# g-benton/Volt

Hardware: AMD Instinct MI355X
Metric: mll_grad_steps_per_s (higher is better)
Workload: dtype f32; 1 GPU; MLL+grad step, N=4096, batch=64 series per GPU, Volatility kernel + EWMA(k=25) mean; series_total=64, parallelism=series-sharded x1, collective=none

## Files before the change

### volt_amd/csrc/tiles.h

```cpp
#pragma once
#include "common.h"
#include "host.h"

namespace volt {


__device__ __forceinline__ float input_elem(const KSource& src, const float* Kb, float add, const float* Ab, int Np,
                                            bool usek, int gi, int gj) {
    if (usek) {
        float v = (gi < src.N && gj < src.N) ? Kb[(int64_t)gi * src.ldk + gj] : 0.f;
        if (gi == gj) v = (gi < src.N) ? v + add : 1.f;
        return v;
    }
    return Ab[(int64_t)gi * Np + gj];
}

template <bool FROMK, int ABL = 0, bool CHASE = false, bool LOCALP = false>
__device__ __forceinline__ void update_body(float* __restrict__ A, int Np, int rowblk, int colblk, int kb0, int kb1,
                                            bool fromk, int b, const KSource& src, float* smem,
                                            bool to_image = false, const Chase* ch = nullptr, bool* ch_ok = nullptr) {
    float* Ab = A + (int64_t)b * Np * Np;
    const float* Arows = Ab + (int64_t)rowblk * TS * Np + (int64_t)kb0 * TS;
    const float* Brows = Ab + (int64_t)colblk * TS * Np + (int64_t)kb0 * TS;
    const int lane = threadIdx.x & 63, wave = threadIdx.x >> 6;
    const int wr = wave >> 1, wc = wave & 1;
    float* C = Ab + (int64_t)rowblk * TS * Np + (int64_t)colblk * TS;
    f32x16 acc[4];
    const bool usek = FROMK && fromk;
    const float add = usek ? ((src.sigma2 ? src.sigma2[b] : 0.f) + src.jitter) : 0.f;
    const float* Kb = usek ? src.K + (int64_t)b * src.bsk : nullptr;
#pragma unroll
    for (int tm = 0; tm < 2; ++tm)
#pragma unroll
        for (int tn = 0; tn < 2; ++tn)
#pragma unroll
            for (int q = 0; q < 16; ++q) {
                const int r = wr * 64 + tm * 32 + accrow(q, lane);
                const int c = wc * 64 + tn * 32 + (lane & 31);
                if (ABL & 1) acc[tm * 2 + tn][q] = 0.f;
                else acc[tm * 2 + tn][q] = -input_elem(src, Kb, add, Ab, Np, usek, rowblk * TS + r, colblk * TS + c);
            }
    gemm_nt_128<0, CHASE, LOCALP>(Arows, Np, Brows, Np, (kb1 - kb0) * (TS / BK), acc, smem, ch, ch_ok);
    if (ABL & 2) {
        float sum = 0.f;
#pragma unroll
        for (int t4 = 0; t4 < 4; ++t4)
#pragma unroll
            for (int q = 0; q < 16; ++q) sum += acc[t4][q];
        C[(int64_t)(threadIdx.x >> 1) * Np + (threadIdx.x & 1)] = sum;
        return;
    }
    if (to_image) {
        __syncthreads();
#pragma unroll
        for (int tm = 0; tm < 2; ++tm)
#pragma unroll
            for (int tn = 0; tn < 2; ++tn)
#pragma unroll
                for (int q = 0; q < 16; ++q) {
                    const int r = wr * 64 + tm * 32 + accrow(q, lane);
                    const int c = wc * 64 + tn * 32 + (lane & 31);
                    smem[r * (TS + 1) + c] = (c <= r) ? -acc[tm * 2 + tn][q] : 0.f;
                }
        return;
    }
#pragma unroll
    for (int tm = 0; tm < 2; ++tm)
#pragma unroll
        for (int tn = 0; tn < 2; ++tn)
#pragma unroll
            for (int q = 0; q < 16; ++q) {
                const int r = wr * 64 + tm * 32 + accrow(q, lane);
                const int c = wc * 64 + tn * 32 + (lane & 31);
                C[(int64_t)r * Np + c] = -acc[tm * 2 + tn][q];
            }
}

constexpr int DT = TS + 1;
constexpr int DIAG_LDS_FLOATS = TS * DT;

__device__ __forceinline__ f32x16 mm32_lds_lds(f32x16 acc, const float* __restrict__ A, const float* __restrict__ B) {
    const int lane = threadIdx.x & 63, l31 = lane & 31, lh = lane >> 5;
    float av[16], bv[16];
#pragma unroll
    for (int s2 = 0; s2 < 16; ++s2) {
        const int kk = 2 * s2 + lh;
        av[s2] = A[l31 * DT + kk];
        bv[s2] = B[kk * DT + l31];
    }
    VOLT_SB();
#pragma unroll
    for (int s2 = 0; s2 < 16; ++s2) acc = __builtin_amdgcn_mfma_f32_32x32x2f32(av[s2], bv[s2], acc, 0, 0, 0);
    return acc;
}
__device__ __forceinline__ f32x16 mm32_lds_reg(f32x16 acc, const float* __restrict__ A, const f32x16& Breg) {
    const int lane = threadIdx.x & 63, l31 = lane & 31, lh = lane >> 5;
    float av[16];
#pragma unroll
    for (int q = 0; q < 16; ++q) av[q] = A[l31 * DT + (q & 3) + 8 * (q >> 2) + 4 * lh];
    VOLT_SB();
#pragma unroll
    for (int q = 0; q < 16; ++q) acc = __builtin_amdgcn_mfma_f32_32x32x2f32(av[q], Breg[q], acc, 0, 0, 0);
    return acc;
}

template <bool NEG>
__device__ __forceinline__ f32x16 mm32_nt(f32x16 acc, const float* __restrict__ A, const float* __restrict__ B) {
    const int lane = threadIdx.x & 63, l31 = lane & 31, lh = lane >> 5;
    float av[16], bv[16];
#pragma unroll
    for (int s2 = 0; s2 < 16; ++s2) {
        const int kk = 2 * s2 + lh;
        av[s2] = A[l31 * DT + kk];
        bv[s2] = B[l31 * DT + kk];
    }
    VOLT_SB();
#pragma unroll
    for (int s2 = 0; s2 < 16; ++s2)
        acc = __builtin_amdgcn_mfma_f32_32x32x2f32(NEG ? -av[s2] : av[s2], bv[s2], acc, 0, 0, 0);
    return acc;
}

__device__ __forceinline__ float lane_bcast(float v, int src) {
    return __int_as_float(__builtin_amdgcn_readlane(__float_as_int(v), src));
}

#define VOLT_RL "v_readlane_b32 "
__device__ __forceinline__ void rl_fma3(float& c0, float& c1, float& c2, float b0, float b1, float b2, float s0,
                                        float s1, float s2, int l0, int l1, int l2) {
    float t0, t1, t2;
    asm volatile(VOLT_RL "%3, %9, %12\n\t" VOLT_RL "%4, %10, %13\n\t" VOLT_RL "%5, %11, %14\n\t"
                 "v_fma_f32 %0, -%6, %3, %0\n\tv_fma_f32 %1, -%7, %4, %1\n\tv_fma_f32 %2, -%8, %5, %2"
                 : "+v"(c0), "+v"(c1), "+v"(c2), "=&s"(t0), "=&s"(t1), "=&s"(t2)
                 : "v"(b0), "v"(b1), "v"(b2), "v"(s0), "v"(s1), "v"(s2), "i"(l0), "i"(l1), "i"(l2));
}
__device__ __forceinline__ void rl_fma2(float& c0, float& c1, float b0, float b1, float s0, float s1, int l0, int l1) {
    float t0, t1;
    asm volatile(VOLT_RL "%2, %6, %8\n\t" VOLT_RL "%3, %7, %9\n\ts_nop 0\n\t"
                 "v_fma_f32 %0, -%4, %2, %0\n\tv_fma_f32 %1, -%5, %3, %1"
                 : "+v"(c0), "+v"(c1), "=&s"(t0), "=&s"(t1)
                 : "v"(b0), "v"(b1), "v"(s0), "v"(s1), "i"(l0), "i"(l1));
}
__device__ __forceinline__ void settle(float& v) { asm volatile("s_nop 0" : "+v"(v)); }

__device__ __forceinline__ void rl_fma1(float& c0, float b0, float s0, int l0) {
    float t0;
    asm volatile(VOLT_RL "%1, %3, %4\n\ts_nop 1\n\tv_fma_f32 %0, -%2, %1, %0"
                 : "+v"(c0), "=&s"(t0)
                 : "v"(b0), "v"(s0), "i"(l0));
}

#define VOLT_STAMP(i)                                                                  \
    do {                                                                               \
        if (STAMP && threadIdx.x == 0) stamps[i] = __builtin_amdgcn_s_memtime();       \
    } while (0)

template <int J0, int J1>
__device__ __forceinline__ void pivots16(float (&a)[32], float (&rv)[32], int& npos) {
    settle(a[J0]);
    float d = lane_bcast(a[J0], J0);
    float rinv = __builtin_amdgcn_rsqf(d);
#pragma unroll
    for (int j = J0; j < J1; ++j) {
        npos += (d > 0.f) ? 1 : 0;
        rv[j] = rinv;
        float l = a[j] * rinv;
        settle(l);
        a[j] = l;
        float rnext = 0.f;
        if (j + 1 < J1) {
            rl_fma1(a[j + 1], l, l, j + 1);
            settle(a[j + 1]);
            d = lane_bcast(a[j + 1], j + 1);
            rnext = __builtin_amdgcn_rsqf(d);
        }
        int c = j + 2;
#pragma unroll
        for (; c + 2 < J1; c += 3) rl_fma3(a[c], a[c + 1], a[c + 2], l, l, l, l, l, l, c, c + 1, c + 2);
        if (c + 1 < J1) rl_fma2(a[c], a[c + 1], l, l, l, l, c, c + 1);
        else if (c < J1) rl_fma1(a[c], l, l, c);
        rinv = rnext;
    }
}
template <int R0, int R1>
__device__ __forceinline__ void invert16(const float (&a)[32], const float (&rv)[32], float (&x)[32], int l31) {
#pragma unroll
    for (int r = R0; r < R1; ++r) x[r] = (r == l31) ? 1.f : 0.f;
#pragma unroll
    for (int m = R0; m < R1; ++m) {
        const float xm = x[m] * rv[m];
        x[m] = xm;
        int r = m + 1;
#pragma unroll
        for (; r + 2 < R1; r += 3) rl_fma3(x[r], x[r + 1], x[r + 2], xm, xm, xm, a[m], a[m], a[m], r, r + 1, r + 2);
        if (r + 1 < R1) rl_fma2(x[r], x[r + 1], xm, xm, a[m], a[m], r, r + 1);
        else if (r < R1) rl_fma1(x[r], xm, a[m], r);
    }
}
__device__ __forceinline__ void wave_lds_fence() {
    __builtin_amdgcn_fence(__ATOMIC_RELEASE, "wavefront");
    __builtin_amdgcn_wave_barrier();
    __builtin_amdgcn_fence(__ATOMIC_ACQUIRE, "wavefront");
}

constexpr int PSC = 17;
constexpr int PIVOT_SCRATCH_FLOATS = 2 * 16 * PSC;
static_assert(DIAG_LDS_FLOATS + 3 * PIVOT_SCRATCH_FLOATS <= 2 * STAGE_FLOATS, "pivot scratch must fit behind the image");

template <bool STAMP = false>
__device__ __forceinline__ void pivot_phase(float* __restrict__ sT, int kb, int prow, float (&a)[32], int& npos,
                                            long long* stamps = nullptr) {
    const int lane = threadIdx.x & 63, wave = threadIdx.x >> 6, l31 = lane & 31, l15 = lane & 15, g = lane >> 4;
    const bool panel = prow >= 0;
    const bool prw = panel && lane >= 32;
    const bool low = !prw && l31 >= 16;
    float* Dk = sT + (32 * kb) * DT + 32 * kb;
    float* Rw = prw ? sT + (32 * prow + l31) * DT + 32 * kb : Dk + l31 * DT;
    float* S21 = sT + DIAG_LDS_FLOATS + wave * PIVOT_SCRATCH_FLOATS;
    float* S22 = S21 + 16 * PSC;
    float rv[32];
#pragma unroll
    for (int c = 0; c < 16; ++c) a[c] = Rw[c];
    if (STAMP && kb == 1) VOLT_STAMP(16);
    pivots16<0, 16>(a, rv, npos);
    if (STAMP && kb == 1) VOLT_STAMP(17);
    {
        float* dst = prw ? Rw : S21 + (l31 & 15) * PSC;
        if (prw || low) {
#pragma unroll
            for (int c = 0; c < 16; ++c) dst[c] = a[c];
        }
    }
    wave_lds_fence();
    float v21[4];
#pragma unroll
    for (int s = 0; s < 4; ++s) v21[s] = S21[l15 * PSC + 4 * s + g];
    {
        f32x4 c22;
#pragma unroll
        for (int q = 0; q < 4; ++q) c22[q] = Dk[(16 + 4 * g + q) * DT + 16 + l15];
#pragma unroll
        for (int s = 0; s < 4; ++s) c22 = __builtin_amdgcn_mfma_f32_16x16x4f32(-v21[s], v21[s], c22, 0, 0, 0);
#pragma unroll
        for (int q = 0; q < 4; ++q) S22[(4 * g + q) * PSC + l15] = c22[q];
    }
    if (panel) {
        float* Pk = sT + (32 * prow) * DT + 32 * kb;
#pragma unroll
        for (int t = 0; t < 2; ++t) {
            f32x4 cp;
#pragma unroll
            for (int q = 0; q < 4; ++q) cp[q] = Pk[(16 * t + 4 * g + q) * DT + 16 + l15];
#pragma unroll
            for (int s = 0; s < 4; ++s)
                cp = __builtin_amdgcn_mfma_f32_16x16x4f32(-Pk[(16 * t + l15) * DT + 4 * s + g], v21[s], cp, 0, 0, 0);
#pragma unroll
            for (int q = 0; q < 4; ++q) Pk[(16 * t + 4 * g + q) * DT + 16 + l15] = cp[q];
        }
    }
    wave_lds_fence();
    if (STAMP && kb == 1) VOLT_STAMP(18);
    {
        const float* src = prw ? Rw + 16 : S22 + (l31 & 15) * PSC;
#pragma unroll
        for (int c = 0; c < 16; ++c) {
            const float t = src[c];
            a[16 + c] = (prw || low) ? t : 0.f;
        }
    }
    if (STAMP && kb == 1) VOLT_STAMP(19);
    pivots16<16, 32>(a, rv, npos);
    if (STAMP && kb == 1) VOLT_STAMP(20);
    if (prw) {
#pragma unroll
        for (int c = 16; c < 32; ++c) Rw[c] = a[c];
    }
}

__device__ __forceinline__ __amdgpu_buffer_rsrc_t w_rsrc(float* W) {
    return __builtin_amdgcn_make_buffer_rsrc((void*)W, 0, TS * TS * 4, 0x00020000);
}
template <int AUX = 0>
__device__ __forceinline__ void w_store(__amdgpu_buffer_rsrc_t rs, int voff, int soff, float v) {
    __builtin_amdgcn_raw_buffer_store_b32(__float_as_uint(v), rs, voff, soff, AUX);
}
template <bool SLABS = false>
__device__ __forceinline__ void x_block(float* __restrict__ sT, int kb, __amdgpu_buffer_rsrc_t rs) {
    constexpr int AUX = SLABS ? AUX_SC1 : 0;
    constexpr bool store00 = SLABS;
    const int lane = threadIdx.x & 63, l15 = lane & 15, g = lane >> 4, h = lane >> 5;
    const bool up = (lane & 16) != 0;
    float* Dk = sT + (32 * kb) * DT + 32 * kb;
    const float* Lh = Dk + (16 * h) * DT + 16 * h;
    float v21[4];
#pragma unroll
    for (int s = 0; s < 4; ++s) v21[s] = Dk[(16 + l15) * DT + 4 * s + g];
    float x[16];
#pragma unroll
    for (int r = 0; r < 16; ++r) {
        float acc = (r == l15) ? 1.f : 0.f;
#pragma unroll
        for (int m = 0; m < r; ++m) acc = __builtin_fmaf(-Lh[r * DT + m], x[m], acc);
        const float d = Lh[r * DT + r];
        const float ri = __builtin_amdgcn_rcpf(d);
        x[r] = acc * __builtin_fmaf(__builtin_fmaf(-d, ri, 1.f), ri, ri);
    }
    wave_lds_fence();
    if (!up) {
#pragma unroll
        for (int r = 0; r < 16; ++r) Dk[(16 * h + r) * DT + 16 * h + l15] = x[r];
    }
    wave_lds_fence();
    f32x4 t21 = {0.f, 0.f, 0.f, 0.f}, r21 = {0.f, 0.f, 0.f, 0.f};
#pragma unroll
    for (int s = 0; s < 4; ++s)
        t21 = __builtin_amdgcn_mfma_f32_16x16x4f32(v21[s], Dk[(4 * s + g) * DT + l15], t21, 0, 0, 0);
#pragma unroll
    for (int q = 0; q < 4; ++q)
        r21 = __builtin_amdgcn_mfma_f32_16x16x4f32(Dk[(16 + l15) * DT + 16 + 4 * g + q], t21[q], r21, 0, 0, 0);
    const int wbase = (32 * kb * TS + 32 * kb) * 4;
#pragma unroll
    for (int q = 0; q < 4; ++q) {
        Dk[(16 + 4 * g + q) * DT + l15] = -r21[q];
        w_store<AUX>(rs, wbase + ((16 + 4 * g) * TS + l15) * 4, q * TS * 4, -r21[q]);
    }
    if (!up || h == 0) {
        const int voff = wbase + (up ? 16 + l15 : (16 * h) * TS + 16 * h + l15) * 4;
        if (kb != 0 || lane != 0 || store00) w_store<AUX>(rs, voff, 0, up ? 0.f : x[0]);
#pragma unroll
        for (int r = 1; r < 16; ++r) w_store<AUX>(rs, voff, r * TS * 4, up ? 0.f : x[r]);
    }
}

__device__ __forceinline__ f32x16 zero16() {
    f32x16 z;
#pragma unroll
    for (int q = 0; q < 16; ++q) z[q] = 0.f;
    return z;
}
__device__ __forceinline__ void w_out(__amdgpu_buffer_rsrc_t rs, int i, int j, float* __restrict__ blk, const f32x16& R) {
    const int lane = threadIdx.x & 63;
    const int voff = ((32 * i + 4 * (lane >> 5)) * TS + 32 * j + (lane & 31)) * 4;
#pragma unroll
    for (int q = 0; q < 16; ++q) {
        w_store(rs, voff, ((q & 3) + 8 * (q >> 2)) * TS * 4, -R[q]);
        if (blk) blk[accrow(q, lane) * DT + (lane & 31)] = -R[q];
    }
}

template <bool STAMP = false, bool SLABS = false, bool LOCALPUB = false>
__device__ __forceinline__ void diag_body(float* __restrict__ A, float* __restrict__ Winv, int* __restrict__ info,
                                          int Np, int k, int b, float* smem, long long* stamps = nullptr,
                                          bool loaded = false, int* ready = nullptr, int ready_val = 0,
                                          int* slab = nullptr, int* pre = nullptr) {
    float* sT = smem;
    VOLT_STAMP(0);
    const int n = Np / TS;
    float* D = A + (int64_t)b * Np * Np + (int64_t)k * TS * Np + (int64_t)k * TS;
    float* W = Winv + ((int64_t)b * n + k) * TS * TS;
    const int tid = threadIdx.x;
    const int lane = tid & 63, wave = tid >> 6, l31 = lane & 31;

    if (!loaded) {
        f32x4 v[TS * TS / 4 / NT];
#pragma unroll
        for (int it = 0; it < TS * TS / 4 / NT; ++it) {
            const int e = tid + it * NT, r = e >> 5, c = (e & 31) * 4;
            v[it] = f32x4{0.f, 0.f, 0.f, 0.f};
            if (c <= r) v[it] = *reinterpret_cast<const f32x4*>(D + (int64_t)r * Np + c);
        }
#pragma unroll
        for (int it = 0; it < TS * TS / 4 / NT; ++it) {
            const int e = tid + it * NT, r = e >> 5, c = (e & 31) * 4;
#pragma unroll
            for (int q = 0; q < 4; ++q) sT[r * DT + c + q] = (c + q <= r) ? v[it][q] : 0.f;
        }
    }
    __syncthreads();
    VOLT_STAMP(1);

    auto blk = [&](int i, int j) { return sT + (32 * i) * DT + 32 * j; };
    const __amdgpu_buffer_rsrc_t wrs = w_rsrc(W);
    auto trail = [&](int i, int j, int m) {
        float* C = blk(i, j);
        f32x16 acc;
#pragma unroll
        for (int q = 0; q < 16; ++q) acc[q] = C[accrow(q, lane) * DT + l31];
        acc = mm32_nt<true>(acc, blk(i, m), blk(j, m));
#pragma unroll
        for (int q = 0; q < 16; ++q) C[accrow(q, lane) * DT + l31] = acc[q];
    };
    auto park_l = [&](int kb, const float (&a)[32]) {
        if (lane < 32) {
            float* Dgk = D + (int64_t)(32 * kb + l31) * Np + 32 * kb;
            float* Dk = blk(kb, kb) + l31 * DT;
#pragma unroll
            for (int c4 = 0; c4 < 8; ++c4) {
                f32x4 v;
#pragma unroll
                for (int q = 0; q < 4; ++q) {
                    v[q] = (4 * c4 + q <= l31) ? a[4 * c4 + q] : 0.f;
                    Dk[4 * c4 + q] = v[q];
                }
                *reinterpret_cast<f32x4*>(Dgk + 4 * c4) = v;
            }
        }
    };
    int bad = 0;
#pragma unroll 1
    for (int kb = 0; kb <= 4; ++kb) {
        float a[32];
        f32x16 P = zero16();
        const int npw = kb > 3 ? 0 : (kb == 3 ? 1 : 3 - kb);
        const int xw = kb == 1 ? 2 : (kb == 4 ? 0 : 1);
        if (wave < npw) {
            int npos = 0;
            pivot_phase<STAMP>(sT, kb, kb < 3 ? kb + 1 + wave : -1, a, npos, stamps);
            if (npos != 32 && bad == 0) {
#pragma unroll
                for (int j = 0; j < 32; ++j) {
                    const float ljj = lane_bcast(a[j], j);
                    if (!(ljj > 0.f) && bad == 0) bad = 32 * kb + j + 1;
                }
            }
            if (kb == 3) park_l(3, a);
        } else if (kb >= 1 && wave == xw) {
            x_block<SLABS>(sT, kb - 1, wrs);
            if (SLABS) {
                const int c = kb - 1, row = lane >> 1, c0 = 16 * (lane & 1);
                const __amdgpu_buffer_rsrc_t drs = __builtin_amdgcn_make_buffer_rsrc((void*)D, 0, 0x7fffffff, 0x00020000);
                for (int i = c + 1; i <= 3; ++i) {
                    const float* src = blk(i, c) + row * DT + c0;
                    const int voff = (int)((((int64_t)(32 * i + row)) * Np + 32 * c + c0) * 4);
#pragma unroll
                    for (int q4 = 0; q4 < 4; ++q4) {
                        const f32x4 v = {src[4 * q4], src[4 * q4 + 1], src[4 * q4 + 2], src[4 * q4 + 3]};
                        __builtin_amdgcn_raw_buffer_store_b128(__builtin_bit_cast(u32x4, v), drs, voff, 16 * q4, AUX_SC1);
                    }
                }
                asm volatile("s_waitcnt vmcnt(0)" ::: "memory");
                if (lane == 0) __hip_atomic_store(slab + c, ready_val, __ATOMIC_RELAXED, __HIP_MEMORY_SCOPE_AGENT);
            }
        } else if (kb == 0) {
            if (SLABS && pre && lane == 0) {
                __builtin_amdgcn_fence(__ATOMIC_RELEASE, "agent");
                __hip_atomic_store(pre, ready_val, __ATOMIC_RELAXED, __HIP_MEMORY_SCOPE_AGENT);
            }
            const u32x4 z = {0u, 0u, 0u, 0u};
            const int voff = ((lane >> 3) * TS + 4 * (lane & 7)) * 4;
#pragma unroll
            for (int i = 0; i < 3; ++i)
#pragma unroll
                for (int j = i + 1; j <= 3; ++j)
#pragma unroll
                    for (int it = 0; it < 4; ++it)
                        __builtin_amdgcn_raw_buffer_store_b128(z, wrs, voff, ((32 * i + 8 * it) * TS + 32 * j) * 4, 0);
        } else if (wave == 3 && kb <= 2) {
            for (int i = kb + 1; i <= 3; ++i)
                for (int j = kb + 1; j <= i; ++j) trail(i, j, kb - 1);
        } else if (kb == 3 && wave == 2) {
            f32x16 S = mm32_lds_lds(zero16(), blk(1, 0), blk(0, 0));
            w_out(wrs, 1, 0, blk(0, 1), mm32_lds_reg(zero16(), blk(1, 1), S));
        } else if (kb == 4 && wave == 1) {
            f32x16 S = mm32_lds_lds(zero16(), blk(2, 0), blk(0, 0));
            S = mm32_lds_lds(S, blk(2, 1), blk(0, 1));
            w_out(wrs, 2, 0, blk(0, 2), mm32_lds_reg(zero16(), blk(2, 2), S));
        } else if (kb == 4 && wave == 2) {
            f32x16 S = mm32_lds_lds(zero16(), blk(2, 1), blk(1, 1));
            w_out(wrs, 2, 1, blk(1, 2), mm32_lds_reg(zero16(), blk(2, 2), S));
            P = mm32_lds_lds(P, blk(3, 1), blk(1, 1));
        } else if (kb == 4 && wave == 3) {
            P = mm32_lds_lds(P, blk(3, 0), blk(0, 0));
            P = mm32_lds_lds(P, blk(3, 1), blk(0, 1));
        }
        if (STAMP && kb == 1 && lane == 0) stamps[21 + wave] = __builtin_amdgcn_s_memtime();
        if (STAMP && kb == 3 && lane == 0) stamps[25 + wave] = __builtin_amdgcn_s_memtime();
        __syncthreads();
        VOLT_STAMP(2 + 2 * kb);
        if (kb == 4) {
            if (wave == 3) {
                P = mm32_lds_lds(P, blk(3, 2), blk(0, 2));
                w_out(wrs, 3, 0, nullptr, mm32_lds_reg(zero16(), blk(3, 3), P));
            } else if (wave == 2) {
                P = mm32_lds_lds(P, blk(3, 2), blk(1, 2));
                w_out(wrs, 3, 1, nullptr, mm32_lds_reg(zero16(), blk(3, 3), P));
            } else if (wave == 1) {
                f32x16 S = mm32_lds_lds(zero16(), blk(3, 2), blk(2, 2));
                w_out(wrs, 3, 2, nullptr, mm32_lds_reg(zero16(), blk(3, 3), S));
            }
        }
        if (kb >= 3) continue;
        if (wave == 0) park_l(kb, a);
        if (kb + 1 + wave <= 3) trail(kb + 1 + wave, kb + 1, kb);
        __syncthreads();
        VOLT_STAMP(3 + 2 * kb);
    }
    if (tid == 0 && bad) atomicCAS(info + b, 0, k * TS + bad);
    VOLT_STAMP(11);
    asm volatile("s_waitcnt vmcnt(0)" ::: "memory");
    __syncthreads();
    VOLT_STAMP(12);
    if (tid == 0) {
        const int bits = __float_as_int(sT[0]);
        if constexpr (LOCALPUB) {
            *reinterpret_cast<volatile int*>(W) = bits ? bits : 0x7fc00000;
        } else {
            __builtin_amdgcn_fence(__ATOMIC_RELEASE, "agent");
            __hip_atomic_store(reinterpret_cast<int*>(W), bits ? bits : 0x7fc00000, __ATOMIC_RELAXED, __HIP_MEMORY_SCOPE_AGENT);
        }
        if (ready) __hip_atomic_store(ready, ready_val, __ATOMIC_RELAXED, __HIP_MEMORY_SCOPE_AGENT);
    }
    VOLT_STAMP(13);
    for (int e = tid; e < TS * TS / 4; e += NT) {
        const int r = e >> 5, c = (e & 31) * 4;
        if ((r >> 5) != (c >> 5)) {
            f32x4 v;
#pragma unroll
            for (int q = 0; q < 4; ++q) v[q] = (c < r) ? sT[r * DT + c + q] : 0.f;
            *reinterpret_cast<f32x4*>(D + (int64_t)r * Np + c) = v;
        }
    }
    VOLT_STAMP(14);
}

constexpr int WLD = TS + 4;


#ifndef VOLT_OUT_NT
#define VOLT_OUT_NT 1
#endif
#if VOLT_OUT_NT
#define VOLT_OUT_STORE(p, v) __builtin_nontemporal_store((v), (p))
#else
#define VOLT_OUT_STORE(p, v) (*(p) = (v))
#endif
__device__ __forceinline__ void tri_store(const f32x16 (&O)[4], float* __restrict__ Out, int64_t ldo) {
    const int lane = threadIdx.x & 63, wave = threadIdx.x >> 6, l31 = lane & 31;
#pragma unroll
    for (int rb = 0; rb < 4; ++rb)
#pragma unroll
        for (int q = 0; q < 16; ++q) {
            const int c = wave * 32 + accrow(q, lane);
            const int r = rb * 32 + l31;
            VOLT_OUT_STORE(Out + (int64_t)c * ldo + r, -O[rb][q]);
        }
}

template <int AUX>
__device__ __forceinline__ void tri_store_aux(const f32x16 (&O)[4], float* __restrict__ Out, int64_t ldo) {
    const int lane = threadIdx.x & 63, wave = threadIdx.x >> 6, l31 = lane & 31;
    const __amdgpu_buffer_rsrc_t rs = __builtin_amdgcn_make_buffer_rsrc((void*)Out, 0, 0x7fffffff, 0x00020000);
    const int voff = (int)((((int64_t)(wave * 32 + 4 * (lane >> 5))) * ldo + l31) * 4);
    const int ld4 = (int)(ldo * 4);
#pragma unroll
    for (int rb = 0; rb < 4; ++rb)
#pragma unroll
        for (int q = 0; q < 16; ++q)
            __builtin_amdgcn_raw_buffer_store_b32(__float_as_uint(-O[rb][q]), rs, voff, ((q & 3) + 8 * (q >> 2)) * ld4 + rb * 128, AUX);
}

template <int AUX>
__device__ __forceinline__ void tri_store_lds(const f32x16 (&O)[4], float* __restrict__ Out, int64_t ldo, float* smem) {
    const int lane = threadIdx.x & 63, wave = threadIdx.x >> 6, l31 = lane & 31, lh = lane >> 5;
    float* mine = smem + wave * 32 * WLD;
#pragma unroll
    for (int rb = 0; rb < 4; ++rb)
#pragma unroll
        for (int q = 0; q < 16; ++q) mine[accrow(q, lane) * WLD + rb * 32 + l31] = -O[rb][q];
    wave_lds_fence();
    const __amdgpu_buffer_rsrc_t rs = __builtin_amdgcn_make_buffer_rsrc((void*)Out, 0, 0x7fffffff, 0x00020000);
    const int voff = (int)((((int64_t)(wave * 32 + lh)) * ldo + 4 * l31) * 4);
    const int ld8 = (int)(ldo * 8);
    f32x4 v[16];
#pragma unroll
    for (int it = 0; it < 16; ++it) v[it] = *reinterpret_cast<const f32x4*>(mine + (2 * it + lh) * WLD + 4 * l31);
    asm volatile("s_waitcnt lgkmcnt(0)" ::: "memory");
    VOLT_SB();
#pragma unroll
    for (int it = 0; it < 16; ++it)
        __builtin_amdgcn_raw_buffer_store_b128(__builtin_bit_cast(u32x4, v[it]), rs, voff, it * ld8, AUX);
    VOLT_SB();
    asm volatile("s_waitcnt vmcnt(0)" ::: "memory");
}

__device__ __forceinline__ void trtri_diag_body(const float* __restrict__ Winv, float* __restrict__ Y, int Np, int i,
                                                int b, TriReduce red, float* smem) {
    const int n = Np / TS;
    float* Yb = Y + (int64_t)b * Np * Np;
    const float* W = Winv + ((int64_t)b * n + i) * TS * TS;
    const int tid = threadIdx.x;
    const int tile_id = i * (i + 1) / 2 + i;
    for (int e = tid; e < TS * TS / 4; e += NT) {
        const int r = e >> 5, c = (e & 31) * 4;
        *reinterpret_cast<f32x4*>(smem + r * WLD + c) = *reinterpret_cast<const f32x4*>(W + r * TS + c);
    }
    __syncthreads();
    float* Yd = Yb + (int64_t)i * TS * Np + (int64_t)i * TS;
    for (int e = tid; e < TS * TS; e += NT) {
        const int c = e >> 7, r = e & 127;
        Yd[(int64_t)c * Np + r] = (r >= c) ? smem[r * WLD + c] : 0.f;
    }
    if (red.rpad) {
        float* sred = smem + TS * WLD;
        float* rv = sred + TS;
        if (tid < TS) rv[tid] = red.rpad[(int64_t)b * Np + i * TS + tid];
        __syncthreads();
        float fz = 0.f, ff = 0.f;
        if (tid < TS) {
            for (int c = 0; c <= tid; ++c) {
                const float y = smem[tid * WLD + c];
                fz += y * rv[c];
                if (i * TS + c < red.N) ff += y * y;
            }
            red.zpart[((int64_t)b * n + i) * Np + i * TS + tid] = fz;
            sred[tid] = ff;
        }
        __syncthreads();
        if (tid < 64) {
            const float tot = wave_sum_f(sred[tid] + sred[tid + 64]);
            if (tid == 0) red.frob[(int64_t)b * (n * (n + 1) / 2) + tile_id] = tot;
        }
    }
}

template <bool WT = false>
__device__ __forceinline__ void trtri_reduce(const f32x16 (&O)[4], int Np, int i, int j, int b, TriReduce red,
                                             float* smem, const float* rvs = nullptr) {
    const int n = Np / TS;
    const int tid = threadIdx.x, lane = tid & 63, wave = tid >> 6, l31 = lane & 31, lh = lane >> 5;
    const int tile_id = i * (i + 1) / 2 + j;
    const float* rv = red.rpad + (int64_t)b * Np + j * TS + wave * 32;
    float rvq[16];
    if (rvs) {
#pragma unroll
        for (int q = 0; q < 16; ++q) rvq[q] = rvs[wave * 32 + accrow(q, lane)];
    } else {
#pragma unroll
        for (int q = 0; q < 16; ++q) rvq[q] = rv[accrow(q, lane)];
    }
    float* sz = smem;
    float ff = 0.f;
#pragma unroll
    for (int rb = 0; rb < 4; ++rb) {
        float cz = 0.f;
#pragma unroll
        for (int q = 0; q < 16; ++q) {
            const float y = -O[rb][q];
            cz += y * rvq[q];
            ff += y * y;
        }
        cz += __shfl_xor(cz, 32);
        if (lh == 0) sz[wave * TS + rb * 32 + l31] = cz;
    }
    ff = wave_sum_f(ff);
    if (lane == 0) sz[4 * TS + wave] = ff;
    __syncthreads();
    if (tid < TS) {
        const float zv = (sz[tid] + sz[TS + tid]) + (sz[2 * TS + tid] + sz[3 * TS + tid]);
        float* zp = red.zpart + ((int64_t)b * n + j) * Np + i * TS + tid;
        if (WT) __hip_atomic_store(zp, zv, __ATOMIC_RELAXED, __HIP_MEMORY_SCOPE_AGENT);
        else *zp = zv;
    }
    if (tid == 0)
        red.frob[(int64_t)b * (n * (n + 1) / 2) + tile_id] = (sz[4 * TS] + sz[4 * TS + 1]) + (sz[4 * TS + 2] + sz[4 * TS + 3]);
}


struct TriJob {
    TriTile t;
    const float* c0;
    bool row_ok, vec_ok;
    float* out;
    int i, j, b;
};

template <bool FROMK>
__device__ __forceinline__ TriJob panel_job(float* __restrict__ A, const float* __restrict__ Winv, int Np, int i, int k,
                                            int b, const KSource& src) {
    const int n = Np / TS;
    float* Ab = A + (int64_t)b * Np * Np;
    const int lane = threadIdx.x & 63, wave = threadIdx.x >> 6, l31 = lane & 31, lh = lane >> 5;
    const bool usek = FROMK && src.K != nullptr;
    TriJob jb;
    jb.t.X = Ab + (int64_t)k * TS * Np;
    jb.t.ldx = Np;
    jb.t.Z = Ab + (int64_t)i * TS * Np;
    jb.t.ldz = Np;
    jb.t.n1 = k * (TS / BK);
    jb.t.W = Winv + ((int64_t)b * n + k) * TS * TS;
    jb.t.flag = reinterpret_cast<const int*>(jb.t.W);
    jb.t.want = 0;
    const int gi = i * TS + wave * 32 + l31;
    const int64_t ld = usek ? src.ldk : (int64_t)Np;
    jb.c0 = (usek ? src.K + (int64_t)b * src.bsk : Ab) + (int64_t)gi * ld + k * TS + 4 * lh;
    jb.row_ok = !usek || gi < src.N;
    jb.vec_ok = !usek || (((src.ldk & 3) == 0) && ((src.bsk & 3) == 0) && (((uintptr_t)src.K & 15) == 0));
    jb.out = Ab + (int64_t)i * TS * Np + (int64_t)k * TS;
    jb.i = -1;
    jb.j = 0;
    jb.b = b;
    return jb;
}

__device__ __forceinline__ TriJob trtri_job(const float* __restrict__ A, const float* __restrict__ Winv,
                                            float* __restrict__ Y, int Np, int i, int j, int b) {
    const int n = Np / TS;
    const float* Ab = A + (int64_t)b * Np * Np;
    float* Yb = Y + (int64_t)b * Np * Np;
    TriJob jb;
    jb.t.X = Ab + (int64_t)i * TS * Np + (int64_t)j * TS;
    jb.t.ldx = Np;
    jb.t.Z = Yb + (int64_t)j * TS * Np + (int64_t)j * TS;
    jb.t.ldz = Np;
    jb.t.n1 = (i - j) * (TS / BK);
    jb.t.W = Winv + ((int64_t)b * n + i) * TS * TS;
    jb.t.flag = nullptr;
    jb.t.want = 0;
    jb.c0 = nullptr;
    jb.row_ok = jb.vec_ok = true;
    jb.out = Yb + (int64_t)j * TS * Np + (int64_t)i * TS;
    jb.i = i;
    jb.j = j;
    jb.b = b;
    return jb;
}

__device__ __forceinline__ void slab_dump(const f32x16 (&acc)[4], float* __restrict__ slab) {
    const __amdgpu_buffer_rsrc_t rs = __builtin_amdgcn_make_buffer_rsrc((void*)slab, 0, TS * TS * 4, 0x00020000);
#pragma unroll
    for (int t4 = 0; t4 < 4; ++t4)
#pragma unroll
        for (int g = 0; g < 4; ++g) {
            f32x4 v;
#pragma unroll
            for (int e = 0; e < 4; ++e) v[e] = acc[t4][4 * g + e];
            __builtin_amdgcn_raw_buffer_store_b128(__builtin_bit_cast(u32x4, v), rs, ((t4 * 4 + g) * NT + (int)threadIdx.x) * 16, 0,
                                                   16 );
        }
}
__device__ __forceinline__ void job_t0(const TriJob& jb, f32x16 (&T)[4]) {
    if (jb.c0 && jb.row_ok && jb.vec_ok) {
#pragma unroll
        for (int tm = 0; tm < 4; ++tm)
#pragma unroll
            for (int g = 0; g < 4; ++g) {
                const f32x4 v = *reinterpret_cast<const f32x4*>(jb.c0 + 32 * tm + 8 * g);
#pragma unroll
                for (int e = 0; e < 4; ++e) T[tm][4 * g + e] = -v[e];
            }
    } else if (jb.c0 && jb.row_ok) {
#pragma unroll
        for (int tm = 0; tm < 4; ++tm)
#pragma unroll
            for (int q = 0; q < 16; ++q) T[tm][q] = -jb.c0[32 * tm + 8 * (q >> 2) + (q & 3)];
    } else {
        zero_acc(T);
    }
}

}
```

Measured before the change: 45.58 steps/s (1 step = MLL+grad over 64 series of N=4096).

## Rebalance panel inverse schedule across waves and use DPP broadcast FMAs

Rewrites the pivot trailing update and the 16x16 triangular solve in x_block to use DPP row_newbcast fused FMA/mul instead of readlane+scalar FMAs, with row values gathered via ds_bpermute. The update is delayed one step so it overlaps the next pivot. The W-block products are rescheduled across waves and kb stages, with partial accumulators parked in unused LDS tiles so work starts earlier and the final post-barrier tail is shorter. It adds LDS round-trips and depends on DPP semantics and the correctness of the lane mapping.

```diff
diff --git a/volt_amd/csrc/tiles.h b/volt_amd/csrc/tiles.h
--- a/volt_amd/csrc/tiles.h
+++ b/volt_amd/csrc/tiles.h
@@ -150,6 +150,18 @@
                  : "v"(b0), "v"(s0), "i"(l0));
 }
 
+__device__ __forceinline__ void fmac_row(float& c, float rep, float m, int n) {
+    asm volatile("v_fmac_f32_dpp %0, -%1, %2 row_newbcast:%3 row_mask:0xf bank_mask:0xf" : "+v"(c) : "v"(rep), "v"(m), "i"(n));
+}
+__device__ __forceinline__ float mul_row(float rep, float m, int n) {
+    float r;
+    asm volatile("v_mul_f32_dpp %0, %1, %2 row_newbcast:%3 row_mask:0xf bank_mask:0xf" : "=v"(r) : "v"(rep), "v"(m), "i"(n));
+    return r;
+}
+__device__ __forceinline__ float rows_of(float v, int src0) {
+    return __int_as_float(__builtin_amdgcn_ds_bpermute(4 * (src0 + (int)(threadIdx.x & 15)), __float_as_int(v)));
+}
+
 #define VOLT_STAMP(i)                                                                  \
     do {                                                                               \
         if (STAMP && threadIdx.x == 0) stamps[i] = __builtin_amdgcn_s_memtime();       \
@@ -160,6 +172,7 @@
     settle(a[J0]);
     float d = lane_bcast(a[J0], J0);
     float rinv = __builtin_amdgcn_rsqf(d);
+    float repp = 0.f, lp = 0.f;
 #pragma unroll
     for (int j = J0; j < J1; ++j) {
         npos += (d > 0.f) ? 1 : 0;
@@ -168,17 +181,21 @@
         settle(l);
         a[j] = l;
         float rnext = 0.f;
+        float rep = 0.f;
+        if (j + 3 < J1) rep = rows_of(l, J0);
         if (j + 1 < J1) {
             rl_fma1(a[j + 1], l, l, j + 1);
             settle(a[j + 1]);
             d = lane_bcast(a[j + 1], j + 1);
             rnext = __builtin_amdgcn_rsqf(d);
         }
-        int c = j + 2;
-#pragma unroll
-        for (; c + 2 < J1; c += 3) rl_fma3(a[c], a[c + 1], a[c + 2], l, l, l, l, l, l, c, c + 1, c + 2);
-        if (c + 1 < J1) rl_fma2(a[c], a[c + 1], l, l, l, l, c, c + 1);
-        else if (c < J1) rl_fma1(a[c], l, l, c);
+        if (j > J0) {
+#pragma unroll
+            for (int c = j + 2; c < J1; ++c) fmac_row(a[c], repp, lp, c - J0);
+        }
+        if (j + 2 < J1) rl_fma1(a[j + 2], l, l, j + 2);
+        repp = rep;
+        lp = l;
         rinv = rnext;
     }
 }
@@ -296,14 +313,22 @@
 #pragma unroll
     for (int s = 0; s < 4; ++s) v21[s] = Dk[(16 + l15) * DT + 4 * s + g];
     float x[16];
+    float lr[16];
+#pragma unroll
+    for (int m = 0; m < 16; ++m) lr[m] = Lh[l15 * DT + m];
+    float rd;
+    {
+        const float d = Lh[l15 * DT + l15];
+        const float ri = __builtin_amdgcn_rcpf(d);
+        rd = __builtin_fmaf(__builtin_fmaf(-d, ri, 1.f), ri, ri);
+        asm volatile("s_nop 1" : "+v"(rd));
+    }
 #pragma unroll
     for (int r = 0; r < 16; ++r) {
         float acc = (r == l15) ? 1.f : 0.f;
 #pragma unroll
-        for (int m = 0; m < r; ++m) acc = __builtin_fmaf(-Lh[r * DT + m], x[m], acc);
-        const float d = Lh[r * DT + r];
-        const float ri = __builtin_amdgcn_rcpf(d);
-        x[r] = acc * __builtin_fmaf(__builtin_fmaf(-d, ri, 1.f), ri, ri);
+        for (int m = 0; m < r; ++m) fmac_row(acc, lr[m], x[m], r);
+        x[r] = mul_row(rd, acc, r);
     }
     wave_lds_fence();
     if (!up) {
@@ -407,10 +432,20 @@
         }
     };
     int bad = 0;
+    auto acc_park = [&](float* U, const f32x16& R) {
+#pragma unroll
+        for (int q = 0; q < 16; ++q) U[accrow(q, lane) * DT + l31] = R[q];
+    };
+    auto acc_back = [&](const float* U) {
+        f32x16 R;
+#pragma unroll
+        for (int q = 0; q < 16; ++q) R[q] = U[accrow(q, lane) * DT + l31];
+        return R;
+    };
 #pragma unroll 1
     for (int kb = 0; kb <= 4; ++kb) {
         float a[32];
-        f32x16 P = zero16();
+        f32x16 S = zero16(), P = zero16();
         const int npw = kb > 3 ? 0 : (kb == 3 ? 1 : 3 - kb);
         const int xw = kb == 1 ? 2 : (kb == 4 ? 0 : 1);
         if (wave < npw) {
@@ -441,6 +476,10 @@
                 asm volatile("s_waitcnt vmcnt(0)" ::: "memory");
                 if (lane == 0) __hip_atomic_store(slab + c, ready_val, __ATOMIC_RELAXED, __HIP_MEMORY_SCOPE_AGENT);
             }
+            if (kb == 3) {
+                wave_lds_fence();
+                w_out(wrs, 2, 1, blk(1, 2), mm32_lds_reg(zero16(), blk(2, 2), acc_back(blk(1, 2))));
+            }
         } else if (kb == 0) {
             if (SLABS && pre && lane == 0) {
                 __builtin_amdgcn_fence(__ATOMIC_RELEASE, "agent");
@@ -458,40 +497,39 @@
         } else if (wave == 3 && kb <= 2) {
             for (int i = kb + 1; i <= 3; ++i)
                 for (int j = kb + 1; j <= i; ++j) trail(i, j, kb - 1);
+        } else if (kb == 2 && wave == 2) {
+            acc_park(blk(0, 3), mm32_lds_lds(zero16(), blk(1, 0), blk(0, 0)));
+            acc_park(blk(1, 3), mm32_lds_lds(zero16(), blk(2, 0), blk(0, 0)));
+            acc_park(blk(2, 3), mm32_lds_lds(zero16(), blk(3, 0), blk(0, 0)));
         } else if (kb == 3 && wave == 2) {
-            f32x16 S = mm32_lds_lds(zero16(), blk(1, 0), blk(0, 0));
-            w_out(wrs, 1, 0, blk(0, 1), mm32_lds_reg(zero16(), blk(1, 1), S));
+            acc_park(blk(1, 3), mm32_lds_lds(acc_back(blk(1, 3)), blk(2, 1), blk(0, 1)));
+            acc_park(blk(2, 3), mm32_lds_lds(acc_back(blk(2, 3)), blk(3, 1), blk(0, 1)));
+        } else if (kb == 4 && wave == 2) {
+            w_out(wrs, 2, 0, blk(0, 2), mm32_lds_reg(zero16(), blk(2, 2), acc_back(blk(1, 3))));
+            wave_lds_fence();
+            P = mm32_lds_lds(acc_back(blk(2, 3)), blk(3, 2), blk(0, 2));
+        } else if (kb == 4 && wave == 3) {
+            P = mm32_lds_lds(zero16(), blk(3, 1), blk(1, 1));
+            P = mm32_lds_lds(P, blk(3, 2), blk(1, 2));
         } else if (kb == 4 && wave == 1) {
-            f32x16 S = mm32_lds_lds(zero16(), blk(2, 0), blk(0, 0));
-            S = mm32_lds_lds(S, blk(2, 1), blk(0, 1));
-            w_out(wrs, 2, 0, blk(0, 2), mm32_lds_reg(zero16(), blk(2, 2), S));
-        } else if (kb == 4 && wave == 2) {
-            f32x16 S = mm32_lds_lds(zero16(), blk(2, 1), blk(1, 1));
-            w_out(wrs, 2, 1, blk(1, 2), mm32_lds_reg(zero16(), blk(2, 2), S));
-            P = mm32_lds_lds(P, blk(3, 1), blk(1, 1));
-        } else if (kb == 4 && wave == 3) {
-            P = mm32_lds_lds(P, blk(3, 0), blk(0, 0));
-            P = mm32_lds_lds(P, blk(3, 1), blk(0, 1));
-        }
+            S = mm32_lds_lds(zero16(), blk(3, 2), blk(2, 2));
+        }
+        if (STAMP && kb == 4 && lane == 0 && wave > 0) stamps[28 + wave] = __builtin_amdgcn_s_memtime();
         if (STAMP && kb == 1 && lane == 0) stamps[21 + wave] = __builtin_amdgcn_s_memtime();
         if (STAMP && kb == 3 && lane == 0) stamps[25 + wave] = __builtin_amdgcn_s_memtime();
         __syncthreads();
         VOLT_STAMP(2 + 2 * kb);
         if (kb == 4) {
-            if (wave == 3) {
-                P = mm32_lds_lds(P, blk(3, 2), blk(0, 2));
-                w_out(wrs, 3, 0, nullptr, mm32_lds_reg(zero16(), blk(3, 3), P));
-            } else if (wave == 2) {
-                P = mm32_lds_lds(P, blk(3, 2), blk(1, 2));
-                w_out(wrs, 3, 1, nullptr, mm32_lds_reg(zero16(), blk(3, 3), P));
-            } else if (wave == 1) {
-                f32x16 S = mm32_lds_lds(zero16(), blk(3, 2), blk(2, 2));
-                w_out(wrs, 3, 2, nullptr, mm32_lds_reg(zero16(), blk(3, 3), S));
-            }
+            if (wave == 2) w_out(wrs, 3, 0, nullptr, mm32_lds_reg(zero16(), blk(3, 3), P));
+            else if (wave == 3) w_out(wrs, 3, 1, nullptr, mm32_lds_reg(zero16(), blk(3, 3), P));
+            else if (wave == 1) w_out(wrs, 3, 2, nullptr, mm32_lds_reg(zero16(), blk(3, 3), S));
         }
         if (kb >= 3) continue;
         if (wave == 0) park_l(kb, a);
         if (kb + 1 + wave <= 3) trail(kb + 1 + wave, kb + 1, kb);
+        if (kb == 2 && wave == 2) w_out(wrs, 1, 0, blk(0, 1), mm32_lds_reg(zero16(), blk(1, 1), acc_back(blk(0, 3))));
+        if (kb == 2 && wave == 1) acc_park(blk(1, 2), mm32_lds_lds(zero16(), blk(2, 1), blk(1, 1)));
+        if (STAMP && kb == 2 && wave == 2 && lane == 0) stamps[15] = __builtin_amdgcn_s_memtime();
         __syncthreads();
         VOLT_STAMP(3 + 2 * kb);
     }
```

Result: no change. 45.59 steps/s (1 step = MLL+grad over 64 series of N=4096), median of 5 (+0.0%).
